# yjh0410/YOLO-Nano

Measured on AMD Instinct MI355X. Metric: images/sec YOLO-Nano-1.0x 416x416 bs=32 inference (network + decode + NMS + host delivery), higher is better.
Workload: dtype f32 (split-f16 MFMA x3, fp32 accumulate); 1 GPU; YOLO-Nano-1.0x 416x416 bs=32/GPU fp32 inference, COCO 80-class head + NMS (BASELINE configs[1]); inputs resident in HBM, kept detections delivered to pinned host memory inside the timed region; global_batch=32, parallelism=image-sharded x1, no collective, rccl_ranks=1, launch_mode=eager, streams_per_gpu=4

## Files before the change

include/yolonano_hip.h:

```cpp
#ifndef YOLONANO_HIP_H
#define YOLONANO_HIP_H

#include <stdint.h>

#ifdef __cplusplus
extern "C" {
#endif

typedef struct yn_handle yn_handle;

enum { YN_BACKBONE_0_5X = 0, YN_BACKBONE_1_0X = 1, YN_BACKBONE_1_5X = 2, YN_BACKBONE_2_0X = 3 };
enum { YN_ACT_NONE = 0, YN_ACT_RELU = 1, YN_ACT_LEAKY = 2 };
enum { YN_F32 = 0, YN_F16 = 1 };
enum { YN_STATUS_OK = 0, YN_STATUS_ERROR = 1, YN_STATUS_RANGE = 2 };

typedef struct yn_config {
    int   input_size;
    int   num_classes;
    int   num_anchors;
    float anchors[18];
    int   backbone;
    float conf_thresh;
    float nms_thresh;
    int   diou_nms;
// ... 4 lines not shown

int  yn_abi_version(void);
int  yn_create(const yn_config* cfg, yn_handle** out);
void yn_destroy(yn_handle* h);
const char* yn_last_error(yn_handle* h);
int  yn_live_device_memory(int64_t* blocks, int64_t* bytes);
int  yn_set_grid(yn_handle* h, int input_size);
int  yn_set_grid_rect(yn_handle* h, int height, int width, int side, int left, int top);
int  yn_grid_shape(yn_handle* h, int* height, int* width, int* side, int* left, int* top);
int  yn_set_stream(yn_handle* h, void* stream);
int  yn_set_thresholds(yn_handle* h, float conf_thresh, float nms_thresh, int diou_nms);
int  yn_num_predictions(yn_handle* h);
int  yn_use_graph(yn_handle* h, int enable);
int  yn_synchronize(yn_handle* h);
int  yn_multi_stream(yn_handle* h, int enable);
int  yn_exact_f32(yn_handle* h, int enable);
int  yn_range_status(yn_handle* h, int* weights_exceed_f16, int* activation_overflow);
int  yn_fuse_decode(yn_handle* h, int enable);
int  yn_group_launch(yn_handle* h, int enable);
int  yn_down_fuse(yn_handle* h, int enable);
int  yn_tail_fuse(yn_handle* h, int enable);
int  yn_nms_prefilter(yn_handle* h, int mode);
int  yn_nms_sweep(yn_handle* h, int enable);
int  yn_nms_sweep_segments(yn_handle* h, int B, int C);
#define YN_NMS_PLAN_B             0
#define YN_NMS_PLAN_N             1
#define YN_NMS_PLAN_C             2
#define YN_NMS_PLAN_FEW           3
#define YN_NMS_PLAN_FUSED         4
#define YN_NMS_PLAN_CHUNKS        5
#define YN_NMS_PLAN_MERGE         6
#define YN_NMS_PLAN_PREFILTER     7
#define YN_NMS_PLAN_PRE_RANKS     8
#define YN_NMS_PLAN_SWEEP         9
#define YN_NMS_PLAN_SWEEP_MAXN    10
#define YN_NMS_PLAN_SWEEP_SLOTS   11
#define YN_NMS_PLAN_SWEEP_SPLIT   12
#define YN_NMS_PLAN_RESOLVE_ONE   13
#define YN_NMS_PLAN_RESOLVE_SPLIT 14
#define YN_NMS_PLAN_DIOU          15
#define YN_NMS_PLAN_INTS          16
int  yn_nms_stages(yn_handle* h, int B, int N, int C, int32_t* plan, int32_t* seg_count, int32_t* seg_off, int32_t* bucket, float* sbox,
                   int32_t* seg_count2, int32_t* bucket2, float* sbox2, int32_t* seg_sparse, int32_t* keep);
int  yn_autotune(yn_handle* h, int enable);
int  yn_set_pw_config(yn_handle* h, int index);
int  yn_tune_save(const char* path, int device);
// ... 306 lines not shown
```

yolo-nano_amd/capi.py:

```python
import ctypes
import os

import numpy as np
import torch

from . import arch

_HERE = os.path.dirname(os.path.abspath(__file__))
LIB_PATH = os.path.join(_HERE, "libyolonano_hip.so")

_vp = ctypes.c_void_p
_i32, _f32 = ctypes.c_int, ctypes.c_float
_i64p = ctypes.POINTER(ctypes.c_int64)

BACKBONE_ID = {"0.5x": 0, "1.0x": 1, "1.5x": 2, "2.0x": 3}


class YnConfig(ctypes.Structure):
    _fields_ = [("input_size", _i32), ("num_classes", _i32), ("num_anchors", _i32),
                ("anchors", _f32 * 18), ("backbone", _i32), ("conf_thresh", _f32), ("nms_thresh", _f32),
                ("diou_nms", _i32), ("max_batch", _i32), ("device", _i32), ("stream", _vp)]


SIGNATURES = {
# ... 11 lines not shown
    "yn_use_graph": (_i32, [_vp, _i32]),
    "yn_synchronize": (_i32, [_vp]),
    "yn_autotune": (_i32, [_vp, _i32]),
    "yn_set_pw_config": (_i32, [_vp, _i32]),
    "yn_tune_save": (_i32, [ctypes.c_char_p, _i32]),
    "yn_tune_load": (_i32, [ctypes.c_char_p, _i32]),
    "yn_allreduce_grads": (_i32, [_vp, _vp]),
    "yn_pw_config_count": (_i32, []),
    "yn_pw_f32_config_count": (_i32, []),
    "yn_unit_chain": (_i32, [_vp, _i32]),
    "yn_chain_pipe": (_i32, [_vp, _i32]),
    "yn_stage_fuse": (_i32, [_vp, _i32, _i32]),
    "yn_pw_pipe": (_i32, [_vp, _i32]),
    "yn_multi_stream": (_i32, [_vp, _i32]),
    "yn_exact_f32": (_i32, [_vp, _i32]),
    "yn_range_status": (_i32, [_vp, ctypes.POINTER(_i32), ctypes.POINTER(_i32)]),
    "yn_fuse_decode": (_i32, [_vp, _i32]),
    "yn_group_launch": (_i32, [_vp, _i32]),
    "yn_down_fuse": (_i32, [_vp, _i32]),
    "yn_tail_fuse": (_i32, [_vp, _i32]),
    "yn_nms_prefilter": (_i32, [_vp, _i32]),
    "yn_nms_sweep": (_i32, [_vp, _i32]),
    "yn_nms_sweep_segments": (_i32, [_vp, _i32, _i32]),
    "yn_nms_stages": (_i32, [_vp, _i32, _i32, _i32] + [_vp] * 10),
    "yn_load_param": (_i32, [_vp, ctypes.c_char_p, _vp, _i64p, _i32]),
    "yn_load_param_dev": (_i32, [_vp, ctypes.c_char_p, _vp, _i64p, _i32]),
    "yn_fold_bn": (_i32, [_vp]),
    "yn_get_folded": (_i32, [_vp, ctypes.c_char_p, _vp, _vp]),
    "yn_forward_raw": (_i32, [_vp, _vp, _i32, _vp, _vp, _vp]),
    "yn_forward_taps": (_i32, [_vp, _vp, _i32, _vp, _vp, _vp]),
    "yn_score_full": (_i32, [_vp, _vp, _vp, _vp, _i32, _vp, _vp]),
    "yn_decode_boxes": (_i32, [_vp, _vp, _i32, _vp]),
    "yn_create_grid": (_i32, [_vp, _i32, _vp, _vp, _vp]),
    "yn_create_grid_rect": (_i32, [_vp, _i32, _i32, _vp, _vp, _vp]),
    "yn_nms": (_i32, [_vp, _vp, _vp, _i32, _f32, _i32, _vp, _vp]),
    "yn_postprocess": (_i32, [_vp, _vp, _vp, _i32, _i32, _i32, _vp, _vp, _vp, _vp, _vp]),
    "yn_infer": (_i32, [_vp, _vp, _i32, _vp, _vp, _vp, _vp, _vp]),
    "yn_pack_detections": (_i32, [_vp, _vp, _vp, _vp, _vp, _i32, _i32, _vp, _vp]),
    "yn_loss": (_i32, [_vp, _vp, _vp, _vp, _vp, _i32, _vp, _vp, _vp, _vp]),
    "yn_loss_heads": (_i32, [_vp, _vp, _vp, _vp, _vp, _i32, _vp, _vp, _vp, _vp]),
    "yn_train_param_count": (ctypes.c_int64, [_vp]),
    "yn_train_param_offset": (_i32, [_vp, ctypes.c_char_p, _i64p, _i64p]),
    "yn_train_bind": (_i32, [_vp, _vp, _vp, _vp, ctypes.c_int64]),
    "yn_train_step": (_i32, [_vp, _vp, _vp, _i32, _f32, _f32, _f32, _f32, _i32, _vp]),
    "yn_read_param": (_i32, [_vp, ctypes.c_char_p, _vp, ctypes.c_int64]),
    "yn_train_forward": (_i32, [_vp, _vp, _i32, _vp, _vp, _vp]),
# ... 315 lines not shown
    def pw_pipe(self, on=True):
        self._ck(self.lib.yn_pw_pipe(self.h, int(bool(on))), "yn_pw_pipe")

    def multi_stream(self, on=True):
        self._ck(self.lib.yn_multi_stream(self.h, int(bool(on))), "yn_multi_stream")

    def exact_f32(self, on=True):
        self._ck(self.lib.yn_exact_f32(self.h, int(bool(on))), "yn_exact_f32")

    def range_status(self):
        w, a = _i32(0), _i32(0)
        self._ck(self.lib.yn_range_status(self.h, ctypes.byref(w), ctypes.byref(a)), "yn_range_status")
        return bool(w.value), bool(a.value)

    def fuse_decode(self, on=True):
        self._ck(self.lib.yn_fuse_decode(self.h, int(on)), "yn_fuse_decode")

    def nms_prefilter(self, mode=1):
        self._ck(self.lib.yn_nms_prefilter(self.h, int(mode)), "yn_nms_prefilter")

    def nms_sweep(self, on=True):
        self._ck(self.lib.yn_nms_sweep(self.h, int(bool(on))), "yn_nms_sweep")

    def nms_sweep_segments(self, B, C):
        return int(self.lib.yn_nms_sweep_segments(self.h, int(B), int(C)))

    NMS_PLAN_FIELDS = ("B", "N", "C", "few", "fused", "chunks", "merge", "prefilter", "pre_ranks", "sweep", "sweep_maxn", "sweep_slots",
                       "sweep_split", "resolve_one", "resolve_split", "diou")

    def nms_stages(self, B, N, C):
        B, N, C = int(B), int(N), int(C)
        plan = np.zeros(len(self.NMS_PLAN_FIELDS), np.int32)
        a = {"seg_count": np.zeros((B, C), np.int32), "seg_off": np.zeros((B, C), np.int32), "bucket": np.zeros((B, N), np.int32),
             "sbox": np.zeros((B, N, 4), np.float32), "seg_count2": np.zeros((B, C), np.int32), "bucket2": np.zeros((B, N), np.int32),
             "sbox2": np.zeros((B, N, 4), np.float32), "seg_sparse": np.zeros((B, C), np.int32), "keep": np.zeros((B, N), np.int32)}
        self._ck(self.lib.yn_nms_stages(self.h, B, N, C, plan.ctypes.data, *[v.ctypes.data for v in a.values()]), "yn_nms_stages")
        a["plan"] = dict(zip(self.NMS_PLAN_FIELDS, (int(v) for v in plan)))
        if not a["plan"]["prefilter"]:
            for k in ("seg_count2", "bucket2", "sbox2", "seg_sparse"):
                a[k] = None
        return a

    def down_fuse(self, on=True):
        self._ck(self.lib.yn_down_fuse(self.h, int(bool(on))), "yn_down_fuse")

    def tail_fuse(self, on=True):
# ... 1017 lines not shown
```

yolo-nano_amd/csrc/kernels_post.hip:

```cpp
#include "yn_device.h"
#include "yn_head_tile_map.h"
#include "yn_prep.h"

namespace ynk {

__device__ __forceinline__ float sigmoid_f(float v) { return 1.0f / (1.0f + expf(-v)); }
__device__ __forceinline__ float exp_le0(float x) { return __builtin_amdgcn_exp2f(x * 1.44269504088896340736f); }

__device__ __forceinline__ void cand_location(const GridInfo& g, int n, int& s, int& cell, int& a)
{
    s = (n >= g.off[2]) ? 2 : ((n >= g.off[1]) ? 1 : 0);
    const int local = n - g.off[s];
    cell = local / g.A;
    a = local - cell * g.A;
}

__device__ __forceinline__ float grid_window_norm(const GridInfo& g, float p, int k)
{
    return (p + (float)((k & 1) ? g.top : g.left)) / (float)g.side;
}

__device__ __forceinline__ void decode_one(const GridInfo& g, int s, int cell, int a, const float* t, float S, float* box, bool normalise)
{
    const int gy = cell / g.w[s], gx = cell - gy * g.w[s];
    const float stride = (float)(8 << s);
// ... 1979 lines not shown

template <bool DIOU>
__global__ __launch_bounds__(64) void single_matrix_kernel(const float4* __restrict__ sbox, int n, float thresh, u64* __restrict__ M)
{
    __shared__ float4 cbox[64];
    __shared__ float carea[64];
    const int T = (n + 63) >> 6;
    const int total = T * (T + 1) / 2;
    for (int t = blockIdx.x; t < total; t += gridDim.x) {
        int rem = t, ri = 0;
        while (rem >= T - ri) { rem -= T - ri; ++ri; }
        matrix_tile<DIOU>(sbox, n, T, ri, ri + rem, thresh, M, cbox, carea);
    }
}

__global__ __launch_bounds__(256) void single_resolve_kernel(const int32_t* __restrict__ ids, int n, const u64* __restrict__ M,
                                                              int32_t* __restrict__ pick_list, int32_t* __restrict__ count)
{
    __shared__ ResolveLds L;
    const int picked = n > 0 ? resolve_segment<2>(ids, n, M, nullptr, pick_list, L) : 0;
    if (threadIdx.x == 0) *count = picked;
}

__global__ __launch_bounds__(1024) void compact_kernel(const float* __restrict__ boxes, const float* __restrict__ scores,
                                                        const int32_t* __restrict__ cls, const int32_t* __restrict__ keep, int N,
                                                        float* __restrict__ out_boxes, float* __restrict__ out_scores,
                                                        int32_t* __restrict__ out_cls, int32_t* __restrict__ out_index,
                                                        int32_t* __restrict__ count, const unsigned* __restrict__ ovf, unsigned* __restrict__ ovf_host)
{
    constexpr int IT = 32;
    __shared__ int wave_sums[IT][16];
    __shared__ int part[8];
    __shared__ int base, total_next;
    const int b = blockIdx.x;
    const int lane = threadIdx.x & 63, wave = threadIdx.x >> 6;
    if (threadIdx.x == 0) base = 0;
    __syncthreads();
    for (int n0 = 0; n0 < N; n0 += IT * 1024) {
        int kf[IT];
#pragma unroll
        for (int it = 0; it < IT; ++it) {
            const int n = n0 + it * 1024 + threadIdx.x;
            kf[it] = keep[(size_t)b * N + (n < N ? n : N - 1)];
        }
        unsigned flags = 0;
        int before[IT];
#pragma unroll
        for (int it = 0; it < IT; ++it) {
            const int n = n0 + it * 1024 + threadIdx.x;
            const int f = (n < N && kf[it]) ? 1 : 0;
            const unsigned long long bal = __ballot(f);
            before[it] = __popcll(bal & ((1ull << lane) - 1ull));
            if (lane == 0) wave_sums[it][wave] = __popcll(bal);
            flags |= (unsigned)f << it;
        }
        __syncthreads();
        int v = 0, incl = 0;
        if (threadIdx.x < IT * 16) {
            v = (&wave_sums[0][0])[threadIdx.x];
            incl = v;
#pragma unroll
            for (int o = 1; o < 64; o <<= 1) { const int t2 = __shfl_up(incl, o); if (lane >= o) incl += t2; }
            if (lane == 63) part[wave] = incl;
        }
        __syncthreads();
        if (threadIdx.x < IT * 16) {
            int add = 0;
#pragma unroll
            for (int w = 0; w < 8; ++w) add += (w < wave) ? part[w] : 0;
            (&wave_sums[0][0])[threadIdx.x] = base + add + incl - v;
            if (threadIdx.x == IT * 16 - 1) total_next = base + add + incl;
        }
        __syncthreads();
#pragma unroll
        for (int g8 = 0; g8 < IT; g8 += 8) {
            float4 bx[8]; float sc[8]; int cl[8];
#pragma unroll
            for (int k = 0; k < 8; ++k) {
                const int it = g8 + k;
                const int n = n0 + it * 1024 + threadIdx.x;
                const size_t src = (size_t)b * N + (((flags >> it) & 1u) ? n : 0);
                bx[k] = *reinterpret_cast<const float4*>(boxes + src * 4);
                sc[k] = scores[src];
                cl[k] = cls[src];
            }
#pragma unroll
            for (int k = 0; k < 8; ++k) {
                const int it = g8 + k;
                if ((flags >> it) & 1u) {
                    const int n = n0 + it * 1024 + threadIdx.x;
                    const size_t dst = (size_t)b * N + wave_sums[it][wave] + before[it];
                    *reinterpret_cast<float4*>(out_boxes + dst * 4) = bx[k];
                    out_scores[dst] = sc[k];
                    out_cls[dst] = cl[k];
                    if (out_index) out_index[dst] = n;
                }
            }
        }
        __syncthreads();
        if (threadIdx.x == 0) base = total_next;
        __syncthreads();
    }
    if (threadIdx.x == 0) {
        const bool flagged = ovf && *ovf;
        count[b] = flagged ? -1 - base : base;
        if (flagged && ovf_host) __hip_atomic_store(ovf_host, 1u, __ATOMIC_RELAXED, __HIP_MEMORY_SCOPE_SYSTEM);
    }
}

int nms_max_segment() { return 64 * YN_RESOLVE_MAX_T; }

__global__ __launch_bounds__(256) void pack_kernel(const float* __restrict__ boxes, const float* __restrict__ scores, const int32_t* __restrict__ cls,
                                                   const int32_t* __restrict__ count, int B, int N, float* __restrict__ rec, int32_t* __restrict__ offsets)
{
    __shared__ int base_s, total_s;
    const int b = blockIdx.x;
    if (threadIdx.x < 64) {
        int mine = 0, all = 0;
        int bad = 0;
        for (int i = threadIdx.x; i < B; i += 64) { int c = count[i]; if (c < 0) { bad = 1; c = -1 - c; } all += c; if (i < b) mine += c; }
        for (int o = 32; o > 0; o >>= 1) { mine += __shfl_xor(mine, o); all += __shfl_xor(all, o); bad |= __shfl_xor(bad, o); }
        if (threadIdx.x == 0) { base_s = mine; total_s = bad ? -1 - all : all; }
    }
    __syncthreads();
    const int base = base_s, k = count[b] < 0 ? -1 - count[b] : count[b];
    if (threadIdx.x == 0) { offsets[b] = base; if (b == 0) offsets[B] = total_s; }
    for (int i = threadIdx.x; i < k; i += 256) {
        const size_t src = (size_t)b * N + i;
        const float4 bx = *reinterpret_cast<const float4*>(boxes + src * 4);
        float* r = rec + (size_t)(base + i) * 6;
        *reinterpret_cast<float2*>(r) = make_float2(bx.x, bx.y);
        *reinterpret_cast<float2*>(r + 2) = make_float2(bx.z, bx.w);
        *reinterpret_cast<float2*>(r + 4) = make_float2(scores[src], (float)cls[src]);
    }
}

void launch_pack(const float* boxes, const float* scores, const int32_t* cls, const int32_t* count, int B, int N, float* rec, int32_t* offsets, hipStream_t s)
{
    hipLaunchKernelGGL(pack_kernel, dim3(B), dim3(256), 0, s, boxes, scores, cls, count, B, N, rec, offsets);
}

size_t nms_pre_sync_words(int B, int N) { return YN_PRE_TICKETS + (size_t)B * YN_PRE_RANKS * pre_sync_words(N); }
size_t nms_matrix_words_per_image(int N, int C)
{
    const size_t Tsum = (size_t)(N + 63) / 64 + C;
    return 64 * (Tsum * (Tsum + 1) / 2);
}

static void set_sort_attr()
{
    static unsigned long long done = 0;
    if (!attr_pending(done)) return;
    (void)hipFuncSetAttribute(reinterpret_cast<const void*>(sort_kernel), hipFuncAttributeMaxDynamicSharedMemorySize, YN_SORT_LARGE * 8);
    (void)hipFuncSetAttribute(reinterpret_cast<const void*>(single_sort_kernel), hipFuncAttributeMaxDynamicSharedMemorySize, YN_SORT_LARGE * 8);
}

const int32_t* launch_nms_bucket_sort(const float* boxes, const float* scores, const int32_t* cls, int B, int N, int C, const NmsWork& wk,
                                      hipStream_t s, const NmsHook* hook, NmsPlan& rec)
{
    set_sort_attr();
    const int large_cap = wk.large_cap;
    auto mark = [&](const char* k) { if (hook && hook->fn) hook->fn(hook->ctx, k); };
// ... 28 lines not shown
            if (N > YN_SORT_SMALL) {
                mark("sort_merge_kernel");
                rec.merge = 1;
                hipLaunchKernelGGL(sort_merge_kernel, dim3((N + 255) / 256, B), dim3(256), 0, s, boxes, wk.seg_count, wk.seg_off, wk.bucket, sbox,
                                   N, C, (const int32_t*)wk.large_list, large_cap, (const u64*)M, wk.matrix_stride);
            }
        } else {
            hipLaunchKernelGGL(sort_kernel, dim3(B, C), dim3(256), YN_SORT_SMALL * 8, s, boxes, scores, wk.seg_count, wk.seg_off, wk.bucket, sbox,
                               N, C, 0, YN_SORT_SMALL, (u64*)nullptr, (size_t)0, (const int32_t*)nullptr, 0, (const int32_t*)wk.seg_order);
            if (N > YN_SORT_SMALL)
                hipLaunchKernelGGL(sort_kernel, dim3(large_cap, B), dim3(1024), YN_SORT_LARGE * 8, s, boxes, scores, wk.seg_count, wk.seg_off, wk.bucket, sbox,
                                   N, C, YN_SORT_SMALL, YN_SORT_LARGE, (u64*)nullptr, (size_t)0, (const int32_t*)wk.large_list, large_cap, (const int32_t*)nullptr);
        }
        if (N > YN_SORT_LARGE && !chunks)
            hipLaunchKernelGGL(sort_kernel, dim3(large_cap, B), dim3(1024), 0, s, boxes, scores, wk.seg_count, wk.seg_off, wk.bucket, sbox,
                               N, C, YN_SORT_LARGE, 1 << 30, M, wk.matrix_stride, (const int32_t*)wk.large_list, large_cap, (const int32_t*)nullptr);
    }
    return seg_order;
}

void launch_nms_compact(const float* boxes, const float* scores, const int32_t* cls, int B, int N, const NmsWork& wk,
                        float* out_boxes, float* out_scores, int32_t* out_cls, int32_t* out_index, int32_t* count, hipStream_t s)
{
    hipLaunchKernelGGL(compact_kernel, dim3(B), dim3(1024), 0, s, boxes, scores, cls, wk.keep, N, out_boxes, out_scores, out_cls, out_index, count, wk.ovf, wk.ovf_host);
}

void launch_nms_pipeline(const float* boxes, const float* scores, const int32_t* cls, int B, int N, int C,
                         float nms_thresh, int diou, const NmsWork& wk,
                         float* out_boxes, float* out_scores, int32_t* out_cls, int32_t* out_index, int32_t* count,
                         hipStream_t s, const NmsHook* hook, NmsPlan* plan)
{
    NmsPlan rec{};
    rec.B = B; rec.N = N; rec.C = C; rec.diou = diou != 0;
    const int large_cap = wk.large_cap;
    auto mark = [&](const char* k) { if (hook && hook->fn) hook->fn(hook->ctx, k); };
    float4* sbox = reinterpret_cast<float4*>(wk.sbox);
    u64* M = reinterpret_cast<u64*>(wk.matrix);
    const int32_t* seg_order = launch_nms_bucket_sort(boxes, scores, cls, B, N, C, wk, s, hook, rec);
    const bool few = rec.few != 0;
    const int32_t* m_count = wk.seg_count;
    const int32_t* m_toff = wk.tile_off;
    const int32_t* m_ids = wk.bucket;
    const float4* m_box = sbox;
    const int prefilter_env = wk.prefilter;
    bool sweep = false;
    int sweep_maxn = 0, sweep_slots = 0;
    if (!diou && wk.sbox2 && (prefilter_env == 2 || (prefilter_env == 1 && B >= 4))) {
// ... 22 lines not shown
        mark("nms_sweep_kernel");
        int sweep_split = (sweep_maxn * 20 <= 64 * 1024 ? 256 : 128) / (B > 0 ? B : 1);
        sweep_split = sweep_split < 2 ? 2 : (sweep_split > 8 ? 8 : sweep_split);
        rec.sweep = 1; rec.sweep_maxn = sweep_maxn; rec.sweep_slots = sweep_slots; rec.sweep_split = sweep_split;
        static unsigned long long attr_sw = 0;
        if (attr_pending(attr_sw)) (void)hipFuncSetAttribute(reinterpret_cast<const void*>(nms_sweep_kernel), hipFuncAttributeMaxDynamicSharedMemorySize, YN_SWEEP_MAXN * 20);
        hipLaunchKernelGGL(nms_sweep_kernel, dim3(B, sweep_split, sweep_slots), dim3(1024), (size_t)sweep_maxn * 20, s, m_box, m_count, wk.seg_off, m_toff, N, C, nms_thresh,
                           M, wk.matrix_stride, (const int32_t*)wk.large_list, large_cap, (const int32_t*)wk.seg_sparse, sweep_maxn);
    }
    mark("resolve_kernel");
    const bool split = N > YN_SORT_SMALL && wk.large_list && large_cap > 0;
    rec.resolve_one = (long)B * C <= 256;
    rec.resolve_split = !rec.resolve_one && split;
    if ((long)B * C <= 256) {
        hipLaunchKernelGGL(resolve_large_kernel, dim3(C, B), dim3(512), 0, s, m_count, wk.seg_off, m_toff, m_ids, N, C, M, wk.matrix_stride,
                           wk.keep, (const int32_t*)nullptr, 0, 0);
    } else {
        hipLaunchKernelGGL(resolve_kernel, dim3(B, C), dim3(256), 0, s, m_count, wk.seg_off, m_toff, m_ids, N, C, M, wk.matrix_stride, wk.keep,
                           split ? YN_SORT_SMALL : 1 << 30, seg_order);
        if (split) hipLaunchKernelGGL(resolve_large_kernel, dim3(B, large_cap), dim3(512), 0, s, m_count, wk.seg_off, m_toff, m_ids, N, C, M, wk.matrix_stride,
                                      wk.keep, (const int32_t*)wk.large_list, large_cap, YN_SORT_SMALL);
    }
    mark("compact_kernel");
    hipLaunchKernelGGL(compact_kernel, dim3(B), dim3(1024), 0, s, boxes, scores, cls, wk.keep, N, out_boxes, out_scores, out_cls, out_index, count, wk.ovf, wk.ovf_host);
    if (plan) *plan = rec;
}

void launch_nms_single(const float* dets, const float* scores, int n, float thresh, int diou,
                       int32_t* ids_scratch, float* sbox_scratch, void* matrix_scratch, int32_t* keep, int32_t* count, hipStream_t s)
{
    set_sort_attr();
    float4* sbox = reinterpret_cast<float4*>(sbox_scratch);
    u64* M = reinterpret_cast<u64*>(matrix_scratch);
    if (n > 0) {
        const int P = nms_pow2(n);
        const int thr = P >= 2048 ? 1024 : 256;
        if (P <= YN_SORT_LARGE) hipLaunchKernelGGL(single_sort_kernel, dim3(1), dim3(thr), (size_t)P * 8, s, dets, scores, n, ids_scratch, sbox, (u64*)nullptr);
        else hipLaunchKernelGGL(single_sort_kernel, dim3(1), dim3(1024), 0, s, dets, scores, n, ids_scratch, sbox, M);
        const int T = (n + 63) / 64;
        int G = T * (T + 1) / 2;
        if (G > 8192) G = 8192;
        if (diou) hipLaunchKernelGGL(single_matrix_kernel<true>, dim3(G), dim3(64), 0, s, sbox, n, thresh, M);
        else      hipLaunchKernelGGL(single_matrix_kernel<false>, dim3(G), dim3(64), 0, s, sbox, n, thresh, M);
    }
    hipLaunchKernelGGL(single_resolve_kernel, dim3(1), dim3(256), 0, s, ids_scratch, n, M, keep, count);
}

// ... 87 lines not shown
```

yolo-nano_amd/csrc/yn_api.hip:

```cpp
#include <hip/hip_runtime.h>

#include <dlfcn.h>

#include <cstdarg>
#include <cstdio>
#include <cstring>
#include <map>
#include <memory>
#include <mutex>
#include <string>
#include <vector>

#include "../../include/yolonano_hip.h"
#include "yn_internal.h"
#include "yn_h16.h"
#include <stdlib.h>

using namespace ynk;

namespace {

thread_local std::string g_create_error;
std::mutex g_tune_mutex;
std::map<std::vector<int>, int> g_pw_tuned;
// ... 110 lines not shown
    hipStream_t stream = nullptr;
    hipStream_t cur = nullptr;
    hipStream_t side[2] = {nullptr, nullptr};
    std::vector<hipEvent_t> fj_events;
    size_t fj_next = 0;
    bool multi_stream = true;
    std::string err;
    std::map<std::string, Param> params;
    std::vector<Layer> layers;
    std::map<std::string, int> by_name;
    std::map<std::string, int> by_conv;
    bool folded = false;
    int stage_ch[3] = {0, 0, 0};
    int head_ch = 0;
    GridInfo grid;
    DevBuf<char> arena;
    size_t arena_bytes = 0, arena_used = 0;
    int arena_S = 0, arena_B = 0;
    DevBuf<float> cand_boxes, cand_scores, nms_sbox, nms_sbox2;
    DevBuf<int32_t> cand_cls, nms_bucket, nms_keep, nms_bucket2;
    DevBuf<int32_t> nms_seg[10];
    DevBuf<unsigned long long> nms_matrix, nms_pre_sync;
    NmsWork nms{};
    DevBuf<float> wbf_box, wbf_score, wbf_ofb, wbf_op, wbf_os;
    DevBuf<int32_t> wbf_votes, wbf_index, wbf_on, wbf_ofounder;
    WbfWork wbf{};
    DevBuf<float> soft_score, soft_spill;
    SoftWork soft{};
    int soft_method = YN_SOFT_OFF;
    float soft_sigma = 0.5f, soft_floor = 0.0f;
    NmsPlan nms_plan{};
    DevBuf<float> heads_buf;
    float* heads_int[3] = {nullptr, nullptr, nullptr};
    float* fwd_only[3] = {nullptr, nullptr, nullptr};
    float* tap_out[3] = {nullptr, nullptr, nullptr};
    DevBuf<float> loss_partial;
    float *tP = nullptr, *tG = nullptr, *tM = nullptr;
    int64_t tN = 0, tN_expected = 0;
    long train_steps = 0;
    std::map<std::string, size_t> toff;
    std::vector<TrainPack> tpacks;
    DevBuf<float> zeros;
    DevBuf<float> train_losses;
    std::vector<TrainGraph> train_graphs; int train_graph_misses = 0; bool train_graph = false; int64_t train_graph_replays = 0;
    int head_fork = -1, head_fork_now = 0, fork_trials = 0;
    hipEvent_t fork_ev[8] = {};
// ... 1283 lines not shown
    if (plan) {
        const int32_t v[YN_NMS_PLAN_INTS] = {p.B, p.N, p.C, p.few, p.fused, p.chunks, p.merge, p.prefilter, p.pre_ranks, p.sweep, p.sweep_maxn, p.sweep_slots,
                                             p.sweep_split, p.resolve_one, p.resolve_split, p.diou};
        for (int i = 0; i < YN_NMS_PLAN_INTS; ++i) plan[i] = v[i];
    }
    auto get = [&](void* dst, const void* src, size_t bytes) {
        if (dst) HIPCHK(h, hipMemcpyAsync(dst, src, bytes, hipMemcpyDeviceToHost, h->stream));
        return 0;
    };
    if (get(seg_count, h->nms.seg_count, seg * 4) || get(seg_off, h->nms.seg_off, seg * 4) || get(bucket, h->nms.bucket, cand * 4) ||
        get(sbox, h->nms.sbox, cand * 16) || get(keep, h->nms.keep, cand * 4)) return 1;
    if (p.prefilter && (get(seg_count2, h->nms.seg_count2, seg * 4) || get(bucket2, h->nms.bucket2, cand * 4) || get(sbox2, h->nms.sbox2, cand * 16) ||
                        get(seg_sparse, h->nms.seg_sparse, seg * 4))) return 1;
    HIPCHK(h, hipStreamSynchronize(h->stream));
    return 0;
}
int yn_nms_sweep(yn_handle* h, int enable)
{
    if (!h) return 1;
    if ((enable != 0) != (h->nms.sweep != 0)) drop_graphs(h);
    h->nms.sweep = enable != 0;
    return 0;
}

int yn_down_fuse(yn_handle* h, int enable)
{
    YN_ENTER(h);
    if ((enable != 0) != h->down_fuse) drop_graphs(h);
    h->down_fuse = enable != 0;
    return 0;
}

int yn_tail_fuse(yn_handle* h, int enable)
{
    YN_ENTER(h);
    if ((enable != 0) != h->tail_fuse) drop_graphs(h);
    h->tail_fuse = enable != 0;
    return 0;
}

int yn_group_launch(yn_handle* h, int enable)
{
    YN_ENTER(h);
    if ((enable != 0) != h->group_launch) drop_graphs(h);
    h->group_launch = enable != 0;
    return 0;
// ... 535 lines not shown
            NmsWork wk = h->nms;
            wk.ovf = exact(h) ? nullptr : h->range_flags + 1;
            wk.ovf_host = exact(h) ? nullptr : h->range_host_dev;
            if (soft)
                launch_soft_pipeline(h->cand_boxes, h->cand_scores, h->cand_cls, B, g.N, g.C, h->soft_method, h->cfg.nms_thresh, h->soft_sigma, h->soft_floor,
                                     wk, h->soft, out_boxes, out_scores, out_cls, out_index, count, h->stream, h->profiling ? &hook : nullptr);
            else
                launch_nms_pipeline(h->cand_boxes, h->cand_scores, h->cand_cls, B, g.N, g.C, h->cfg.nms_thresh, h->cfg.diou_nms, wk,
                                    out_boxes, out_scores, out_cls, out_index, count, h->stream, h->profiling ? &hook : nullptr, &h->nms_plan);
            delete ctx.cur;
        }
        HIPCHK(h, hipGetLastError());
        return 0;
    });
}

int yn_pack_detections(yn_handle* h, const float* out_boxes, const float* out_scores, const int32_t* out_cls, const int32_t* count,
                       int B, int N, float* rec_dev, int32_t* offsets_dev)
{
    YN_ENTER(h);
    if (B <= 0 || N <= 0 || !out_boxes || !out_scores || !out_cls || !count || !rec_dev || !offsets_dev)
        return fail(h, "yn_pack_detections: bad arguments");
    if (int rp = range_pending(h, "yn_pack_detections")) return rp;
    launch_pack(out_boxes, out_scores, out_cls, count, B, N, rec_dev, offsets_dev, h->stream);
    HIPCHK(h, hipGetLastError());
    return 0;
}

static int ensure_loss(yn_handle* h, int B)
{
    const size_t need = (size_t)loss_num_blocks(h->grid, B) * 4;
    if (need <= h->loss_partial.cap()) return 0;
    HIPCHK(h, hipStreamSynchronize(h->stream));
    drop_train_graphs(h);
    HIPCHK(h, h->loss_partial.reserve(need));
    return 0;
}

int yn_loss(yn_handle* h, const float* conf, const float* cls, const float* txtytwth, const float* target, int B,
            float* losses, float* g_conf, float* g_cls, float* g_txtytwth)
{
    YN_ENTER(h);
    if (need_square_grid(h, "yn_loss")) return 1;
    if (B <= 0) return fail(h, "yn_loss: batch must be positive");
    if ((g_conf != nullptr) != (g_cls != nullptr) || (g_conf != nullptr) != (g_txtytwth != nullptr))
        return fail(h, "yn_loss: pass all three gradient buffers or none");
    if (ensure_loss(h, B)) return 1;
// ... 752 lines not shown
    }
    if (st[0]) {
        int worst = 0;
        for (int b = 0; b < n; ++b) if (st[MERGE_STATE + b] > cap) { worst = b; break; }
        return fail(h, "%s: the merge list of %s %d needs %d rows, list_capacity is %d (the largest list of the batch needs %d)", who, unit, worst,
                    st[MERGE_STATE + worst], cap, st[1]);
    }
    if (st[3]) {
        const int worst = 4095 - (st[3] >> 19);
        return fail(h, "%s: %s %d was appended %d rows whose class is not an integer in 0..%d", who, unit, worst, st[3] & ((1 << 19) - 1), C - 1);
    }
    const bool soft_on = rule == YN_MERGE_NMS && soft != YN_SOFT_OFF;
    if (rule == YN_MERGE_WBF ? ensure_wbf(h, n, cap, C) : (soft_on ? ensure_soft(h, n, cap, C) : ensure_post(h, n, cap, C))) return 1;
    NmsWork wk = h->nms;
    wk.ovf = nullptr; wk.ovf_host = nullptr;
    if (rule == YN_MERGE_WBF) {
        const int e = expected > 0 ? expected : (default_expected > 0 ? default_expected : 1);
        launch_wbf_pipeline(lb, ls, lc, n, cap, C, nms_thresh, e, wk, h->wbf, mb, ms, mc, nullptr, nullptr, nullptr, mcount, h->stream);
    } else if (soft_on) {
        launch_soft_pipeline(lb, ls, lc, n, cap, C, soft, nms_thresh, soft_sigma, soft_floor, wk, h->soft, mb, ms, mc, nullptr, mcount, h->stream);
    } else {
        launch_nms_pipeline(lb, ls, lc, n, cap, C, nms_thresh, 0, wk, mb, ms, mc, nullptr, mcount, h->stream);
    }
    launch_pack(mb, ms, mc, mcount, n, cap, rec, offsets, h->stream);
    HIPCHK(h, hipGetLastError());
    last_n = n;
    return 0;
}

int MergeLists::empty_result(yn_handle* h, int n)
{
    HIPCHK(h, hipMemsetAsync(offsets, 0, (size_t)(n + 1) * sizeof(int32_t), h->stream));
    last_n = n; lists_n = n; total = 0;
    return 0;
}

int MergeLists::result(const float** rec_dev, const int32_t** offsets_dev, int32_t* total_out)
{
    if (last_n < 0) return 1;
    if (rec_dev) *rec_dev = rec;
    if (offsets_dev) *offsets_dev = offsets;
    if (total_out) {
        if (total < 0) {
            DeviceScope on(device);
            int32_t v = 0;
            if (hipMemcpyAsync(&v, offsets + last_n, sizeof(int32_t), hipMemcpyDeviceToHost, last_stream) != hipSuccess ||
                hipStreamSynchronize(last_stream) != hipSuccess)
// ... 638 lines not shown
```

yolo-nano_amd/csrc/yn_internal.h:

```cpp
#pragma once
#include <hip/hip_runtime.h>
#include <stdint.h>

#include <string>

#include "yn_devbuf.h"
#include "yn_head_tile_map.h"

namespace ynk {

extern bool g_log_lds;
void note_launch_lds(const char* kernel, size_t dyn_lds, unsigned threads);
}
#undef hipLaunchKernelGGL
#define hipLaunchKernelGGL(kernelName, numBlocks, numThreads, memPerBlock, streamId, ...)                                            \
    do {                                                                                                                              \
        if (ynk::g_log_lds) ynk::note_launch_lds(#kernelName, (size_t)(memPerBlock), (unsigned)(dim3(numThreads).x * dim3(numThreads).y)); \
        hipLaunchKernelGGLInternal((kernelName), numBlocks, numThreads, memPerBlock, streamId, __VA_ARGS__);                         \
    } while (0)
namespace ynk {

struct GemmArgs {
    const float* in;   int in_ld;   int in_off;
    const float* in2;  int resample;
// ... 147 lines not shown
                        float* boxes, float* scores, int32_t* cls, hipStream_t s);
struct NmsWork {
    int32_t* seg_count;
    int32_t* seg_off;
    int32_t* tile_off;
    int32_t* bucket;
    int32_t* keep;
    float*   sbox;
    void*    matrix;
    size_t   matrix_stride;
    int32_t* large_list;
    int32_t* bucket2; float* sbox2;
    int32_t* seg_count2; int32_t* tile_off2;
    int32_t* seg_order;
    int32_t* seg_sparse;
    int32_t* work_off;
    void*    pre_sync;
    int32_t* ctr;
    int      prefilter;
    int      sweep;
    int      large_cap;
    const unsigned* ovf;
    unsigned* ovf_host;
};
size_t nms_matrix_words_per_image(int N, int C);
size_t nms_pre_sync_words(int B, int N);
int nms_max_segment();
struct NmsHook { void (*fn)(void* ctx, const char* kernel); void* ctx; };
struct NmsPlan {
    int B, N, C;
    int few;
    int fused;
    int chunks;
    int merge;
    int prefilter;
    int pre_ranks;
    int sweep;
    int sweep_maxn, sweep_slots, sweep_split;
    int resolve_one;
    int resolve_split;
    int diou;
};
void launch_nms_pipeline(const float* boxes, const float* scores, const int32_t* cls, int B, int N, int C,
                         float nms_thresh, int diou, const NmsWork& wk,
                         float* out_boxes, float* out_scores, int32_t* out_cls, int32_t* out_index, int32_t* count,
                         hipStream_t s, const NmsHook* hook = nullptr, NmsPlan* plan = nullptr);
void launch_pack(const float* boxes, const float* scores, const int32_t* cls, const int32_t* count, int B, int N, float* rec, int32_t* offsets, hipStream_t s);
const int32_t* launch_nms_bucket_sort(const float* boxes, const float* scores, const int32_t* cls, int B, int N, int C, const NmsWork& wk,
                                      hipStream_t s, const NmsHook* hook, NmsPlan& rec);
void launch_nms_compact(const float* boxes, const float* scores, const int32_t* cls, int B, int N, const NmsWork& wk,
                        float* out_boxes, float* out_scores, int32_t* out_cls, int32_t* out_index, int32_t* count, hipStream_t s);

constexpr int YN_WBF_LDS_CLUSTERS = 512;
struct WbfWork {
    float* wbox;
    float* wscore;
    int32_t* wvotes;
    int32_t* windex;
    float* ofb; float* op;
    float* os; int32_t* on; int32_t* ofounder;
};
void launch_wbf_pipeline(const float* boxes, const float* scores, const int32_t* cls, int B, int N, int C, float iou_thresh, int expected,
                         const NmsWork& wk, const WbfWork& ww, float* out_boxes, float* out_scores, int32_t* out_cls, int32_t* out_index,
                         int32_t* out_votes, int32_t* assign, int32_t* count, hipStream_t s);
long long wbf_cost(long long n_rows, long long n_clusters);
void launch_fuse_append(const float* rec, const int32_t* offsets, int B, int C, int cap, float weight, float* lboxes, float* lscores, int32_t* lcls,
                        int32_t* state, hipStream_t st);

constexpr int YN_SOFT_LDS_ROWS = 2048;
constexpr int SOFT_HARD = 1, SOFT_LINEAR = 2, SOFT_GAUSSIAN = 3;
// ... 244 lines not shown
```

Before: 53920 images/s.

## Split NMS compact and pack kernels into per-image slices across many blocks

The compaction kernel, which ran one 1024-thread block per image, now launches a 2D grid of 256-thread blocks, each handling a slice of the keep array. Each slice first recounts the kept flags before its start with vectorized int4 ballots to find its output offset. The pack kernel is sliced the same way, and a new API sets the slice counts, with an automatic default aimed at about 512 blocks. This is meant to fill the GPU during the tail stages when B=32 gives only 32 blocks, at the cost of redundant prefix counting in later slices.

Result: no change. 54050 images/s, median of 6 (+0.2%).

```diff
diff --git a/include/yolonano_hip.h b/include/yolonano_hip.h
--- a/include/yolonano_hip.h
+++ b/include/yolonano_hip.h
@@ -50,6 +50,7 @@
 int  yn_tail_fuse(yn_handle* h, int enable);
 int  yn_nms_prefilter(yn_handle* h, int mode);
 int  yn_nms_sweep(yn_handle* h, int enable);
+int  yn_nms_tail_slices(yn_handle* h, int compact_slices, int pack_slices);
 int  yn_nms_sweep_segments(yn_handle* h, int B, int C);
 #define YN_NMS_PLAN_B             0
 #define YN_NMS_PLAN_N             1
diff --git a/yolo-nano_amd/capi.py b/yolo-nano_amd/capi.py
--- a/yolo-nano_amd/capi.py
+++ b/yolo-nano_amd/capi.py
@@ -57,6 +57,7 @@
     "yn_nms_prefilter": (_i32, [_vp, _i32]),
     "yn_nms_sweep": (_i32, [_vp, _i32]),
     "yn_nms_sweep_segments": (_i32, [_vp, _i32, _i32]),
+    "yn_nms_tail_slices": (_i32, [_vp, _i32, _i32]),
     "yn_nms_stages": (_i32, [_vp, _i32, _i32, _i32] + [_vp] * 10),
     "yn_load_param": (_i32, [_vp, ctypes.c_char_p, _vp, _i64p, _i32]),
     "yn_load_param_dev": (_i32, [_vp, ctypes.c_char_p, _vp, _i64p, _i32]),
@@ -418,6 +419,9 @@
     def nms_sweep(self, on=True):
         self._ck(self.lib.yn_nms_sweep(self.h, int(bool(on))), "yn_nms_sweep")
 
+    def nms_tail_slices(self, compact_slices=0, pack_slices=0):
+        self._ck(self.lib.yn_nms_tail_slices(self.h, int(compact_slices), int(pack_slices)), "yn_nms_tail_slices")
+
     def nms_sweep_segments(self, B, C):
         return int(self.lib.yn_nms_sweep_segments(self.h, int(B), int(C)))
 
diff --git a/yolo-nano_amd/csrc/kernels_post.hip b/yolo-nano_amd/csrc/kernels_post.hip
--- a/yolo-nano_amd/csrc/kernels_post.hip
+++ b/yolo-nano_amd/csrc/kernels_post.hip
@@ -1,6 +1,7 @@
 #include "yn_device.h"
 #include "yn_head_tile_map.h"
 #include "yn_prep.h"
+#include "yn_nms_tail.h"
 
 namespace ynk {
 
@@ -2026,88 +2027,111 @@
     if (threadIdx.x == 0) *count = picked;
 }
 
-__global__ __launch_bounds__(1024) void compact_kernel(const float* __restrict__ boxes, const float* __restrict__ scores,
-                                                        const int32_t* __restrict__ cls, const int32_t* __restrict__ keep, int N,
-                                                        float* __restrict__ out_boxes, float* __restrict__ out_scores,
-                                                        int32_t* __restrict__ out_cls, int32_t* __restrict__ out_index,
-                                                        int32_t* __restrict__ count, const unsigned* __restrict__ ovf, unsigned* __restrict__ ovf_host)
-{
-    constexpr int IT = 32;
-    __shared__ int wave_sums[IT][16];
-    __shared__ int part[8];
-    __shared__ int base, total_next;
-    const int b = blockIdx.x;
+__global__ __launch_bounds__(256) void compact_kernel(const float* __restrict__ boxes, const float* __restrict__ scores,
+                                                       const int32_t* __restrict__ cls, const int32_t* __restrict__ keep, int N, int L,
+                                                       float* __restrict__ out_boxes, float* __restrict__ out_scores,
+                                                       int32_t* __restrict__ out_cls, int32_t* __restrict__ out_index,
+                                                       int32_t* __restrict__ count, const unsigned* __restrict__ ovf, unsigned* __restrict__ ovf_host)
+{
+    constexpr int IT = 8;
+    constexpr int RJ = 12;
+    __shared__ int wave_sums[IT][4];
+    __shared__ int before_s[4];
+    __shared__ int pass_total;
+    const int s = blockIdx.x, b = blockIdx.y;
     const int lane = threadIdx.x & 63, wave = threadIdx.x >> 6;
-    if (threadIdx.x == 0) base = 0;
-    __syncthreads();
-    for (int n0 = 0; n0 < N; n0 += IT * 1024) {
+    const int start = s * L, end = start + L < N ? start + L : N;
+    const int32_t* __restrict__ kb = keep + (size_t)b * N;
+    int run = 0;
+    if (start > 0) {
+        const int a0 = (int)((4u - (unsigned)((reinterpret_cast<uintptr_t>(kb) >> 2) & 3u)) & 3u);
+        const int G = (start - a0) >> 2;
+        const int t0 = a0 + 4 * G;
+        const int4* __restrict__ kv = reinterpret_cast<const int4*>(kb + a0);
+        int cnt = 0;
+        for (int g0 = 0; g0 < G; g0 += RJ * 256) {
+            int4 v[RJ];
+#pragma unroll
+            for (int j = 0; j < RJ; ++j) {
+                const int g = g0 + j * 256 + (int)threadIdx.x;
+                v[j] = kv[g < G ? g : G - 1];
+            }
+#pragma unroll
+            for (int j = 0; j < RJ; ++j) {
+                const bool in = g0 + j * 256 + (int)threadIdx.x < G;
+                cnt += __popcll(__ballot(in && v[j].x)) + __popcll(__ballot(in && v[j].y)) + __popcll(__ballot(in && v[j].z)) + __popcll(__ballot(in && v[j].w));
+            }
+        }
+        int e = -1;
+        if ((int)threadIdx.x < a0) e = threadIdx.x;
+        else if (threadIdx.x >= 3 && threadIdx.x < 6 && t0 + (int)threadIdx.x - 3 < start) e = t0 + (int)threadIdx.x - 3;
+        const int ef = kb[e >= 0 ? e : 0];
+        cnt += __popcll(__ballot(e >= 0 && ef));
+        if (lane == 0) before_s[wave] = cnt;
+        __syncthreads();
+        run = before_s[0] + before_s[1] + before_s[2] + before_s[3];
+    }
+    for (int n0 = start; n0 < end; n0 += IT * 256) {
         int kf[IT];
 #pragma unroll
         for (int it = 0; it < IT; ++it) {
-            const int n = n0 + it * 1024 + threadIdx.x;
-            kf[it] = keep[(size_t)b * N + (n < N ? n : N - 1)];
+            const int n = n0 + it * 256 + (int)threadIdx.x;
+            kf[it] = kb[n < end ? n : end - 1];
         }
         unsigned flags = 0;
         int before[IT];
 #pragma unroll
         for (int it = 0; it < IT; ++it) {
-            const int n = n0 + it * 1024 + threadIdx.x;
-            const int f = (n < N && kf[it]) ? 1 : 0;
+            const int n = n0 + it * 256 + (int)threadIdx.x;
+            const int f = (n < end && kf[it]) ? 1 : 0;
             const unsigned long long bal = __ballot(f);
             before[it] = __popcll(bal & ((1ull << lane) - 1ull));
             if (lane == 0) wave_sums[it][wave] = __popcll(bal);
             flags |= (unsigned)f << it;
         }
         __syncthreads();
-        int v = 0, incl = 0;
-        if (threadIdx.x < IT * 16) {
-            v = (&wave_sums[0][0])[threadIdx.x];
-            incl = v;
-#pragma unroll
-            for (int o = 1; o < 64; o <<= 1) { const int t2 = __shfl_up(incl, o); if (lane >= o) incl += t2; }
-            if (lane == 63) part[wave] = incl;
+        if (wave == 0) {
+            const int v = lane < IT * 4 ? (&wave_sums[0][0])[lane] : 0;
+            int incl = v;
+#pragma unroll
+            for (int o = 1; o < IT * 4; o <<= 1) { const int t2 = __shfl_up(incl, o); if (lane >= o) incl += t2; }
+            if (lane < IT * 4) (&wave_sums[0][0])[lane] = run + incl - v;
+            if (lane == IT * 4 - 1) pass_total = incl;
         }
         __syncthreads();
-        if (threadIdx.x < IT * 16) {
-            int add = 0;
-#pragma unroll
-            for (int w = 0; w < 8; ++w) add += (w < wave) ? part[w] : 0;
-            (&wave_sums[0][0])[threadIdx.x] = base + add + incl - v;
-            if (threadIdx.x == IT * 16 - 1) total_next = base + add + incl;
-        }
-        __syncthreads();
-#pragma unroll
-        for (int g8 = 0; g8 < IT; g8 += 8) {
-            float4 bx[8]; float sc[8]; int cl[8];
-#pragma unroll
-            for (int k = 0; k < 8; ++k) {
-                const int it = g8 + k;
-                const int n = n0 + it * 1024 + threadIdx.x;
-                const size_t src = (size_t)b * N + (((flags >> it) & 1u) ? n : 0);
-                bx[k] = *reinterpret_cast<const float4*>(boxes + src * 4);
-                sc[k] = scores[src];
-                cl[k] = cls[src];
-            }
-#pragma unroll
-            for (int k = 0; k < 8; ++k) {
-                const int it = g8 + k;
-                if ((flags >> it) & 1u) {
-                    const int n = n0 + it * 1024 + threadIdx.x;
-                    const size_t dst = (size_t)b * N + wave_sums[it][wave] + before[it];
-                    *reinterpret_cast<float4*>(out_boxes + dst * 4) = bx[k];
-                    out_scores[dst] = sc[k];
-                    out_cls[dst] = cl[k];
-                    if (out_index) out_index[dst] = n;
+#pragma unroll
+        for (int g4 = 0; g4 < IT; g4 += 4) {
+            if (n0 + g4 * 256 < end) {
+                float4 bx[4]; float sc[4]; int cl[4];
+#pragma unroll
+                for (int k = 0; k < 4; ++k) {
+                    const int it = g4 + k;
+                    const int n = n0 + it * 256 + (int)threadIdx.x;
+                    const size_t src = (size_t)b * N + (((flags >> it) & 1u) ? n : 0);
+                    bx[k] = *reinterpret_cast<const float4*>(boxes + src * 4);
+                    sc[k] = scores[src];
+                    cl[k] = cls[src];
+                }
+#pragma unroll
+                for (int k = 0; k < 4; ++k) {
+                    const int it = g4 + k;
+                    if ((flags >> it) & 1u) {
+                        const int n = n0 + it * 256 + (int)threadIdx.x;
+                        const size_t dst = (size_t)b * N + wave_sums[it][wave] + before[it];
+                        *reinterpret_cast<float4*>(out_boxes + dst * 4) = bx[k];
+                        out_scores[dst] = sc[k];
+                        out_cls[dst] = cl[k];
+                        if (out_index) out_index[dst] = n;
+                    }
                 }
             }
         }
+        run += pass_total;
         __syncthreads();
-        if (threadIdx.x == 0) base = total_next;
-        __syncthreads();
-    }
-    if (threadIdx.x == 0) {
+    }
+    if (s == (int)gridDim.x - 1 && threadIdx.x == 0) {
         const bool flagged = ovf && *ovf;
-        count[b] = flagged ? -1 - base : base;
+        count[b] = flagged ? -1 - run : run;
         if (flagged && ovf_host) __hip_atomic_store(ovf_host, 1u, __ATOMIC_RELAXED, __HIP_MEMORY_SCOPE_SYSTEM);
     }
 }
@@ -2115,10 +2139,13 @@
 int nms_max_segment() { return 64 * YN_RESOLVE_MAX_T; }
 
 __global__ __launch_bounds__(256) void pack_kernel(const float* __restrict__ boxes, const float* __restrict__ scores, const int32_t* __restrict__ cls,
-                                                   const int32_t* __restrict__ count, int B, int N, float* __restrict__ rec, int32_t* __restrict__ offsets)
+                                                   const int32_t* __restrict__ count, int B, int N, int L, float* __restrict__ rec, int32_t* __restrict__ offsets)
 {
     __shared__ int base_s, total_s;
-    const int b = blockIdx.x;
+    const int s = blockIdx.x, b = blockIdx.y;
+    const int k = count[b] < 0 ? -1 - count[b] : count[b];
+    const int first = s * L, last = first + L < k ? first + L : k;
+    if (s > 0 && first >= k) return;
     if (threadIdx.x < 64) {
         int mine = 0, all = 0;
         int bad = 0;
@@ -2127,9 +2154,9 @@
         if (threadIdx.x == 0) { base_s = mine; total_s = bad ? -1 - all : all; }
     }
     __syncthreads();
-    const int base = base_s, k = count[b] < 0 ? -1 - count[b] : count[b];
-    if (threadIdx.x == 0) { offsets[b] = base; if (b == 0) offsets[B] = total_s; }
-    for (int i = threadIdx.x; i < k; i += 256) {
+    const int base = base_s;
+    if (s == 0 && threadIdx.x == 0) { offsets[b] = base; if (b == 0) offsets[B] = total_s; }
+    for (int i = first + threadIdx.x; i < last; i += 256) {
         const size_t src = (size_t)b * N + i;
         const float4 bx = *reinterpret_cast<const float4*>(boxes + src * 4);
         float* r = rec + (size_t)(base + i) * 6;
@@ -2139,9 +2166,11 @@
     }
 }
 
-void launch_pack(const float* boxes, const float* scores, const int32_t* cls, const int32_t* count, int B, int N, float* rec, int32_t* offsets, hipStream_t s)
-{
-    hipLaunchKernelGGL(pack_kernel, dim3(B), dim3(256), 0, s, boxes, scores, cls, count, B, N, rec, offsets);
+void launch_pack(const float* boxes, const float* scores, const int32_t* cls, const int32_t* count, int B, int N, float* rec, int32_t* offsets, hipStream_t s,
+                 int slices)
+{
+    const NmsTailCut cut = nms_tail_cut(B, N, slices);
+    hipLaunchKernelGGL(pack_kernel, dim3(cut.slices, B), dim3(256), 0, s, boxes, scores, cls, count, B, N, cut.len, rec, offsets);
 }
 
 size_t nms_pre_sync_words(int B, int N) { return YN_PRE_TICKETS + (size_t)B * YN_PRE_RANKS * pre_sync_words(N); }
@@ -2216,7 +2245,9 @@
 void launch_nms_compact(const float* boxes, const float* scores, const int32_t* cls, int B, int N, const NmsWork& wk,
                         float* out_boxes, float* out_scores, int32_t* out_cls, int32_t* out_index, int32_t* count, hipStream_t s)
 {
-    hipLaunchKernelGGL(compact_kernel, dim3(B), dim3(1024), 0, s, boxes, scores, cls, wk.keep, N, out_boxes, out_scores, out_cls, out_index, count, wk.ovf, wk.ovf_host);
+    const NmsTailCut cut = nms_tail_cut(B, N, wk.compact_slices);
+    hipLaunchKernelGGL(compact_kernel, dim3(cut.slices, B), dim3(256), 0, s, boxes, scores, cls, wk.keep, N, cut.len, out_boxes, out_scores, out_cls, out_index, count,
+                       wk.ovf, wk.ovf_host);
 }
 
 void launch_nms_pipeline(const float* boxes, const float* scores, const int32_t* cls, int B, int N, int C,
@@ -2285,7 +2316,7 @@
                                       wk.keep, (const int32_t*)wk.large_list, large_cap, YN_SORT_SMALL);
     }
     mark("compact_kernel");
-    hipLaunchKernelGGL(compact_kernel, dim3(B), dim3(1024), 0, s, boxes, scores, cls, wk.keep, N, out_boxes, out_scores, out_cls, out_index, count, wk.ovf, wk.ovf_host);
+    launch_nms_compact(boxes, scores, cls, B, N, wk, out_boxes, out_scores, out_cls, out_index, count, s);
     if (plan) *plan = rec;
 }
 
diff --git a/yolo-nano_amd/csrc/yn_api.hip b/yolo-nano_amd/csrc/yn_api.hip
--- a/yolo-nano_amd/csrc/yn_api.hip
+++ b/yolo-nano_amd/csrc/yn_api.hip
@@ -156,6 +156,7 @@
     DevBuf<int32_t> nms_seg[10];
     DevBuf<unsigned long long> nms_matrix, nms_pre_sync;
     NmsWork nms{};
+    int pack_slices = 0;
     DevBuf<float> wbf_box, wbf_score, wbf_ofb, wbf_op, wbf_os;
     DevBuf<int32_t> wbf_votes, wbf_index, wbf_on, wbf_ofounder;
     WbfWork wbf{};
@@ -1485,6 +1486,15 @@
     h->nms.sweep = enable != 0;
     return 0;
 }
+int yn_nms_tail_slices(yn_handle* h, int compact_slices, int pack_slices)
+{
+    YN_ENTER(h);
+    if (compact_slices < 0 || pack_slices < 0) return fail(h, "yn_nms_tail_slices: (%d, %d): a slice count is 0 (automatic) or positive", compact_slices, pack_slices);
+    if (compact_slices != h->nms.compact_slices) drop_graphs(h);
+    h->nms.compact_slices = compact_slices;
+    h->pack_slices = pack_slices;
+    return 0;
+}
 
 int yn_down_fuse(yn_handle* h, int enable)
 {
@@ -2066,7 +2076,7 @@
     if (B <= 0 || N <= 0 || !out_boxes || !out_scores || !out_cls || !count || !rec_dev || !offsets_dev)
         return fail(h, "yn_pack_detections: bad arguments");
     if (int rp = range_pending(h, "yn_pack_detections")) return rp;
-    launch_pack(out_boxes, out_scores, out_cls, count, B, N, rec_dev, offsets_dev, h->stream);
+    launch_pack(out_boxes, out_scores, out_cls, count, B, N, rec_dev, offsets_dev, h->stream, h->pack_slices);
     HIPCHK(h, hipGetLastError());
     return 0;
 }
@@ -2865,7 +2875,7 @@
     } else {
         launch_nms_pipeline(lb, ls, lc, n, cap, C, nms_thresh, 0, wk, mb, ms, mc, nullptr, mcount, h->stream);
     }
-    launch_pack(mb, ms, mc, mcount, n, cap, rec, offsets, h->stream);
+    launch_pack(mb, ms, mc, mcount, n, cap, rec, offsets, h->stream, h->pack_slices);
     HIPCHK(h, hipGetLastError());
     last_n = n;
     return 0;
diff --git a/yolo-nano_amd/csrc/yn_internal.h b/yolo-nano_amd/csrc/yn_internal.h
--- a/yolo-nano_amd/csrc/yn_internal.h
+++ b/yolo-nano_amd/csrc/yn_internal.h
@@ -193,6 +193,7 @@
     int      large_cap;
     const unsigned* ovf;
     unsigned* ovf_host;
+    int      compact_slices;
 };
 size_t nms_matrix_words_per_image(int N, int C);
 size_t nms_pre_sync_words(int B, int N);
@@ -216,7 +217,8 @@
                          float nms_thresh, int diou, const NmsWork& wk,
                          float* out_boxes, float* out_scores, int32_t* out_cls, int32_t* out_index, int32_t* count,
                          hipStream_t s, const NmsHook* hook = nullptr, NmsPlan* plan = nullptr);
-void launch_pack(const float* boxes, const float* scores, const int32_t* cls, const int32_t* count, int B, int N, float* rec, int32_t* offsets, hipStream_t s);
+void launch_pack(const float* boxes, const float* scores, const int32_t* cls, const int32_t* count, int B, int N, float* rec, int32_t* offsets, hipStream_t s,
+                 int slices);
 const int32_t* launch_nms_bucket_sort(const float* boxes, const float* scores, const int32_t* cls, int B, int N, int C, const NmsWork& wk,
                                       hipStream_t s, const NmsHook* hook, NmsPlan& rec);
 void launch_nms_compact(const float* boxes, const float* scores, const int32_t* cls, int B, int N, const NmsWork& wk,
diff --git a/yolo-nano_amd/csrc/yn_nms_tail.h b/yolo-nano_amd/csrc/yn_nms_tail.h
--- /dev/null
+++ b/yolo-nano_amd/csrc/yn_nms_tail.h
@@ -0,0 +1,21 @@
+#pragma once
+
+struct NmsTailCut {
+    int slices;
+    int len;
+};
+
+inline NmsTailCut nms_tail_cut(int B, int N, int want)
+{
+    const long n = N > 0 ? N : 1, b = B > 0 ? B : 1;
+    long S = want;
+    if (S <= 0) {
+        S = (512 + b - 1) / b;
+        const long cap = (n + 1023) / 1024;
+        if (S > cap) S = cap;
+    }
+    const long most = (n + 255) / 256;
+    if (S > most) S = most;
+    const long L = ((n + S - 1) / S + 255) / 256 * 256;
+    return NmsTailCut{(int)((n + L - 1) / L), (int)L};
+}
```
